# ctu-mrs/vofod

Measured on AMD Instinct MI355X. Metric: LiDAR frames/sec (131k-pt OS1-128) at 1/2/4/8 MI355X + HBM roofline %, higher is better.
Workload: dtype f32; 1 GPU; os1-128 128x1024 scans, 0.25 m voxels, batched process_scan (configs[1] scan shape in configs[3]'s batched form); points_per_frame=131072, map_voxels=19480981, map_warm_scans=96, gpu_max_hw_queues=4

## Files before the change

### vofod_amd/csrc/kernels_classify.h

```cpp
#pragma once
#include <hip/hip_runtime.h>

#include "common.h"

namespace vc
{
using namespace vk;

constexpr int EX_MAX_R = 32;
constexpr int EX_SIDE = 2 * EX_MAX_R + 1;
constexpr uint32_t EX_CELLS = EX_SIDE * EX_SIDE * EX_SIDE;
constexpr uint32_t EX_WORDS = (EX_CELLS + 31) / 32;
constexpr uint32_t EX_MAX_JOBS = 1024;

struct ExploreJob
{
  uint32_t frame;
  uint32_t n_members;
  uint32_t member_off;
  int32_t R;
  int32_t box_lo[3], box_hi[3];
  uint32_t result_slot;
};

struct ExploreResult
{
  uint32_t floating;
  uint32_t overflow;
  double conf_sum;
};

struct ExploreParams
{
  float thr_unknown, thr_ground, frontier_value;
  double ray_score;
  int32_t no_update;
  uint32_t stack_cap;
};

__device__ __forceinline__ void wave_sync()
{
  __builtin_amdgcn_fence(__ATOMIC_RELEASE, "workgroup");
  __builtin_amdgcn_wave_barrier();
  __builtin_amdgcn_fence(__ATOMIC_ACQUIRE, "workgroup");
}

__device__ __forceinline__ uint32_t pack_rel(int dx, int dy, int dz) { return static_cast<uint32_t>((dx + 128) | ((dy + 128) << 8) | ((dz + 128) << 16)); }

__device__ __forceinline__ void explore_frame(const ExploreParams& ep, const MapGeom& mg, const ExploreJob* __restrict__ jobs, const uint32_t jb, const uint32_t je, const int* __restrict__ members,
                                              float* __restrict__ map, unsigned long long* __restrict__ overlay_all, uint32_t* __restrict__ stack_all, uint32_t* __restrict__ explored_all,
                                              uint32_t* __restrict__ touched_all, uint32_t* __restrict__ ovl_list_all, uint32_t* __restrict__ ovl_count_all, ExploreResult* __restrict__ results,
                                              uint32_t* __restrict__ visited_all, const uint32_t slot, uint8_t* s_float, uint8_t* s_walk)
{
  const int lane = threadIdx.x & 63;
  if (jb == je)
    return;
  const uint64_t ovl_words = (mg.n + 63) >> 6;
  unsigned long long* overlay = overlay_all + static_cast<uint64_t>(slot) * ovl_words;
  uint32_t* stack = stack_all + static_cast<uint64_t>(slot) * ep.stack_cap;
  uint32_t* explored = explored_all + static_cast<uint64_t>(slot) * ep.stack_cap;
  uint32_t* ovl_list = ovl_list_all + static_cast<uint64_t>(slot) * ep.stack_cap;
  uint32_t* touched = touched_all + static_cast<uint64_t>(slot) * ep.stack_cap;
  uint32_t* visited = visited_all + static_cast<uint64_t>(slot) * EX_WORDS;

  auto map_read = [&](uint64_t li) -> float {
    const float mv = map[li];
    if (!ep.no_update)
      return mv;
    const unsigned long long ow = __hip_atomic_load(&overlay[li >> 6], __ATOMIC_RELAXED, __HIP_MEMORY_SCOPE_AGENT);
    return ((ow >> (li & 63)) & 1ull) ? ep.frontier_value : mv;
  };

  for (uint32_t j = jb; j < je; j++)
  {
    const ExploreJob job = jobs[j];
    bool floating = true;
    uint32_t overflow = 0;
    const float max_voxel_dist = static_cast<float>(job.R);
    uint32_t m = 0;
    while (m < job.n_members && floating)
    {
      {
        const uint32_t mm = m + lane;
        int kind = 0;
        if (mm < job.n_members)
        {
          const int sx_ = members[3 * (job.member_off + mm)], sy_ = members[3 * (job.member_off + mm) + 1], sz_ = members[3 * (job.member_off + mm) + 2];
          if (sx_ <= 0 || sy_ <= 0 || sz_ <= 0 || sx_ >= mg.sx - 1 || sy_ >= mg.sy - 1 || sz_ >= mg.sz - 1)
            kind = 1;
          else
          {
            const float sv = map_read((static_cast<uint64_t>(sz_) * mg.sy + sy_) * mg.sx + sx_);
            kind = sv > ep.thr_ground ? 1 : (sv > ep.thr_unknown ? 2 : 0);
          }
        }
        const unsigned long long need = __ballot(kind != 0);
        if (!need)
        {
          m += 64;
          continue;
        }
        const int first = __ffsll(static_cast<long long>(need)) - 1;
        m += first;
        if (__shfl(kind, first) == 1)
        {
          floating = false;
          break;
        }
      }
      const int ox = members[3 * (job.member_off + m)], oy = members[3 * (job.member_off + m) + 1], oz = members[3 * (job.member_off + m) + 2];
      if (job.R - 1 >= 1 && job.R - 1 <= 31)
      {
        const int len = job.R - 1;
        float wv[3];
        bool win[3];
        const uint64_t li0 = (static_cast<uint64_t>(oz) * mg.sy + oy) * mg.sx + ox;
#pragma unroll
        for (int u = 0; u < 3; u++)
        {
          const int e = lane + 64 * u, q = e >> 5, d = (e & 31) + 1;
          const int ax = ox + (q == 0 ? d : q == 3 ? -d : 0), ay = oy + (q == 1 ? d : q == 4 ? -d : 0), az = oz + (q == 2 ? d : q == 5 ? -d : 0);
          win[u] = d <= len && ax >= 0 && ax <= mg.sx - 1 && ay >= 0 && ay <= mg.sy - 1 && az >= 0 && az <= mg.sz - 1;
          wv[u] = map_read(win[u] ? (static_cast<uint64_t>(az) * mg.sy + ay) * mg.sx + ax : li0);
        }
#pragma unroll
        for (int u = 0; u < 3; u++)
          s_walk[lane + 64 * u] = !win[u] ? 0 : (wv[u] > ep.thr_ground ? 2 : (wv[u] > ep.thr_unknown ? 1 : 0));
        wave_sync();
        bool walk_ok = false;
        if (lane < 6)
        {
          walk_ok = true;
          for (int d = 1; d <= len; d++)
          {
            const uint8_t st = s_walk[(lane << 5) + d - 1];
            if (st == 2)
              break;
            if (st == 0)
            {
              walk_ok = false;
              break;
            }
          }
        }
        const bool any_walk = __ballot(walk_ok) != 0ull;
        wave_sync();
        if (any_walk)
        {
          floating = false;
          break;
        }
      }
      uint32_t n_stack = 1, n_expl = 0, n_touched = 1;
      if (lane == 0)
      {
        stack[0] = pack_rel(0, 0, 0);
        const uint32_t c = (EX_MAX_R * EX_SIDE + EX_MAX_R) * EX_SIDE + EX_MAX_R;
        atomicOr(&visited[c >> 5], 1u << (c & 31));
        touched[0] = c;
      }
      wave_sync();
      bool connected = false;
      while (n_stack > 0 && !connected)
      {
        const uint32_t take = min(n_stack, 64u);
        const uint32_t base = n_stack - take;
        n_stack = base;
        bool have = static_cast<uint32_t>(lane) < take;
        int dx = 0, dy = 0, dz = 0;
        float val = 0.0f;
        if (have)
        {
          const uint32_t e = stack[base + lane];
          dx = static_cast<int>(e & 255u) - 128;
          dy = static_cast<int>((e >> 8) & 255u) - 128;
          dz = static_cast<int>((e >> 16) & 255u) - 128;
          val = map_read((static_cast<uint64_t>(oz + dz) * mg.sy + (oy + dy)) * mg.sx + (ox + dx));
        }
        const bool ground = have && val > ep.thr_ground;
        const bool unknown = have && !ground && val > ep.thr_unknown;
        const int md = abs(dx) + abs(dy) + abs(dz);
        const bool rim = unknown && static_cast<float>(md) == max_voxel_dist - 1.0f;
        if (__ballot(ground || rim))
        {
          connected = true;
          break;
        }
        const unsigned long long um = __ballot(unknown);
        if (unknown)
        {
          const uint32_t pos = n_expl + __popcll(um & ((1ull << lane) - 1ull));
          if (pos < ep.stack_cap)
            explored[pos] = pack_rel(dx, dy, dz);
        }
        n_expl += __popcll(um);
        uint32_t mine[6];
        int n_mine = 0;
        if (unknown)
        {
          const int nb[6][3] = {{1, 0, 0}, {0, 1, 0}, {0, 0, 1}, {-1, 0, 0}, {0, -1, 0}, {0, 0, -1}};
          uint32_t oldw[6], bitq[6];
          bool okq[6];
#pragma unroll
          for (int q = 0; q < 6; q++)
          {
            const int tx = dx + nb[q][0], ty = dy + nb[q][1], tz = dz + nb[q][2];
            const int ax = ox + tx, ay = oy + ty, az = oz + tz;
            const int tmd = abs(tx) + abs(ty) + abs(tz);
            okq[q] = !(ax < 0 || ax > mg.sx - 1 || ay < 0 || ay > mg.sy - 1 || az < 0 || az > mg.sz - 1) && static_cast<float>(tmd) <= max_voxel_dist;
            const uint32_t c = okq[q] ? ((tz + EX_MAX_R) * EX_SIDE + (ty + EX_MAX_R)) * EX_SIDE + (tx + EX_MAX_R) : 0u;
            bitq[q] = 1u << (c & 31);
            oldw[q] = okq[q] ? atomicOr(&visited[c >> 5], bitq[q]) : 0xffffffffu;
          }
#pragma unroll
          for (int q = 0; q < 6; q++)
            if (okq[q] && !(oldw[q] & bitq[q]))
              mine[n_mine++] = pack_rel(dx + nb[q][0], dy + nb[q][1], dz + nb[q][2]);
        }
        uint32_t incl = static_cast<uint32_t>(n_mine);
#pragma unroll
        for (int s = 1; s < 64; s <<= 1)
        {
          const uint32_t t = __shfl_up(incl, s);
          if (lane >= s)
            incl += t;
        }
        const uint32_t total = __shfl(incl, 63);
        uint32_t at = n_stack + incl - n_mine;
        uint32_t tat = n_touched + incl - n_mine;
        for (int q = 0; q < n_mine; q++, at++, tat++)
        {
          if (at < ep.stack_cap)
            stack[at] = mine[q];
          else
            overflow = 1;
          if (tat < ep.stack_cap)
          {
            const int tx = static_cast<int>(mine[q] & 255u) - 128, ty = static_cast<int>((mine[q] >> 8) & 255u) - 128, tz = static_cast<int>((mine[q] >> 16) & 255u) - 128;
            touched[tat] = ((tz + EX_MAX_R) * EX_SIDE + (ty + EX_MAX_R)) * EX_SIDE + (tx + EX_MAX_R);
          }
        }
        n_stack = min(n_stack + total, ep.stack_cap);
        n_touched += total;
        wave_sync();
      }
      wave_sync();
      if (n_touched <= ep.stack_cap)
      {
        for (uint32_t e = lane; e < n_touched; e += 64)
          __hip_atomic_store(&visited[touched[e] >> 5], 0u, __ATOMIC_RELAXED, __HIP_MEMORY_SCOPE_AGENT);
      }
      else
        for (uint32_t w = lane; w < EX_WORDS; w += 64)
          __hip_atomic_store(&visited[w], 0u, __ATOMIC_RELAXED, __HIP_MEMORY_SCOPE_AGENT);
      __threadfence_block();
      wave_sync();
      if (connected)
      {
        floating = false;
        break;
      }
      for (uint32_t e = lane; e < min(n_expl, ep.stack_cap); e += 64)
      {
        const uint32_t pk = explored[e];
        const int dx = static_cast<int>(pk & 255u) - 128, dy = static_cast<int>((pk >> 8) & 255u) - 128, dz = static_cast<int>((pk >> 16) & 255u) - 128;
        const uint64_t li = (static_cast<uint64_t>(oz + dz) * mg.sy + (oy + dy)) * mg.sx + (ox + dx);
        if (ep.no_update)
        {
          const unsigned long long bit = 1ull << (li & 63);
          const unsigned long long old = atomicOr(&overlay[li >> 6], bit);
          if (!(old & bit))
          {
            const uint32_t pos = atomicAdd(&ovl_count_all[slot], 1u);
            if (pos < ep.stack_cap)
              ovl_list[pos] = static_cast<uint32_t>(li >> 6);
          }
        }
        else
          map[li] = ep.frontier_value;
      }
      __threadfence_block();
      wave_sync();
      m++;
    }
    if (lane == 0)
    {
      s_float[j - jb] = floating ? 1 : 0;
      results[job.result_slot].floating = floating ? 1u : 0u;
      results[job.result_slot].overflow = overflow;
      results[job.result_slot].conf_sum = 0.0;
    }
  }
  __threadfence_block();
  wave_sync();

  for (uint32_t j = jb; j < je; j++)
  {
    const ExploreJob job = jobs[j];
    if (!s_float[j - jb])
      continue;
    const int nx = job.box_hi[0] - job.box_lo[0] + 1, ny = job.box_hi[1] - job.box_lo[1] + 1, nz = job.box_hi[2] - job.box_lo[2] + 1;
    const uint32_t cells = static_cast<uint32_t>(nx) * ny * nz;
    double acc = 0.0;
    for (uint32_t c = lane; c < cells; c += 64)
    {
      const int x = job.box_lo[0] + static_cast<int>(c % nx), y = job.box_lo[1] + static_cast<int>((c / nx) % ny), z = job.box_lo[2] + static_cast<int>(c / (nx * ny));
      bool is_member = false;
      for (uint32_t m = 0; m < job.n_members; m++)
      {
        const int* o = &members[3 * (job.member_off + m)];
        is_member |= (o[0] == x && o[1] == y && o[2] == z);
      }
      const float v = is_member ? static_cast<float>(ep.ray_score) : map_read((static_cast<uint64_t>(z) * mg.sy + y) * mg.sx + x);
      acc += 1.0 - static_cast<double>(v) / ep.ray_score;
    }
#pragma unroll
    for (int s = 32; s > 0; s >>= 1)
      acc += __shfl_xor(acc, s);
    if (lane == 0)
      results[job.result_slot].conf_sum = acc;
  }
  if (ep.no_update)
  {
    wave_sync();
    const uint32_t n = __hip_atomic_load(&ovl_count_all[slot], __ATOMIC_RELAXED, __HIP_MEMORY_SCOPE_AGENT);
    if (n <= ep.stack_cap)
      for (uint32_t e = lane; e < n; e += 64)
        overlay[ovl_list[e]] = 0ull;
    else
      for (uint64_t w = lane; w < ovl_words; w += 64)
        overlay[w] = 0ull;
    wave_sync();
    if (lane == 0)
      ovl_count_all[slot] = 0;
  }
}

__global__ __attribute__((amdgpu_waves_per_eu(8, 8))) __launch_bounds__(64) void k_explore(const ExploreParams ep, const MapGeom mg, const ExploreJob* __restrict__ jobs, const uint32_t* __restrict__ job_begin, const uint32_t* __restrict__ job_end,
                                                const int* __restrict__ members, float* __restrict__ map, unsigned long long* __restrict__ overlay_all,
                                                uint32_t* __restrict__ stack_all, uint32_t* __restrict__ explored_all, uint32_t* __restrict__ touched_all,
                                                uint32_t* __restrict__ ovl_list_all, uint32_t* __restrict__ ovl_count_all, ExploreResult* __restrict__ results, uint32_t* __restrict__ visited_all)
{
  __shared__ uint8_t s_float[EX_MAX_JOBS];
  __shared__ uint8_t s_walk[6 * 32];
  const uint32_t slot = blockIdx.x;
  explore_frame(ep, mg, jobs, job_begin[slot], job_end[slot], members, map, overlay_all, stack_all, explored_all, touched_all, ovl_list_all, ovl_count_all, results, visited_all, slot, s_float, s_walk);
}

}
```

### vofod_amd/csrc/kernels_tail.h

```cpp
#pragma once
#include <hip/hip_runtime.h>

#include "host_tail.h"
#include "kernels_classify.h"
#include "kernels_voxelize.h"

namespace vtd
{

#ifndef TAIL_WPB_DEF
#define TAIL_WPB_DEF 8
#endif
constexpr int TAIL_WPB = TAIL_WPB_DEF;
#if TAIL_WPB_DEF >= 16
#define TAIL_OCC_ATTR
#else
#define TAIL_OCC_ATTR __attribute__((amdgpu_waves_per_eu(5, 5)))
#endif
using namespace vk;

constexpr int TAIL_STAGE = 512;
constexpr int TP_THREADS = 256;
constexpr int TP_MAXM = TAIL_MAXM;
constexpr int TP_MAXC = TAIL_MAXC;
constexpr int TP_MAXD = 16;

using vt::TailParams;

struct TailCluster
{
  uint32_t root, n_members;
  float obb_center[3];
  int32_t job;
};

struct DetRaw
{
  uint32_t root, n_points;
  float center[3];
  uint32_t pad;
  double conf_sum;
};

struct FrameDets
{
  uint32_t n;
  uint32_t fallback;
  int32_t status;
  uint32_t n_jobs;
  DetRaw d[TP_MAXD];
};

enum : uint32_t { TAIL_FB_MEMBERS = 1u, TAIL_FB_CLUSTERS = 2u, TAIL_FB_RADIUS = 4u, TAIL_FB_DETS = 8u, TAIL_FB_EXPLORE = 16u };

__device__ __forceinline__ uint32_t rank_in_wave(bool flag, int lane, uint32_t& count)
{
  const unsigned long long m = __ballot(flag);
  count = __popcll(m);
  return __popcll(m & ((1ull << lane) - 1ull));
}

__device__ __forceinline__ void put_header(FrameDets& out, FrameDets* hout, uint32_t f, uint32_t n, uint32_t fb, int32_t status, uint32_t n_jobs)
{
  out.n = n;
  out.fallback = fb;
  out.status = status;
  out.n_jobs = n_jobs;
  if (hout)
  {
    hout[f].n = n;
    hout[f].fallback = fb;
    hout[f].status = status;
    hout[f].n_jobs = n_jobs;
  }
}

__device__ __forceinline__ void write_records(const TailCluster& tc, const vc::ExploreResult* __restrict__ results, int lane, FrameDets& out, FrameDets* hout, uint32_t f, uint32_t& n, uint32_t& fb)
{
  bool det = false, bad = false;
  double conf = 0.0;
  if (tc.job >= 0)
  {
    const vc::ExploreResult r = results[tc.job];
    det = r.floating != 0u;
    bad = r.overflow != 0u;
    conf = r.conf_sum;
  }
  const uint32_t pos = rank_in_wave(det, lane, n);
  const unsigned long long bm = __ballot(bad);
  if (det && pos < TP_MAXD)
  {
    DetRaw d;
    d.root = tc.root;
    d.n_points = tc.n_members;
    for (int q = 0; q < 3; q++)
      d.center[q] = tc.obb_center[q];
    d.pad = 0;
    d.conf_sum = conf;
    out.d[pos] = d;
    if (hout)
      hout[f].d[pos] = d;
  }
  fb = (n > TP_MAXD ? TAIL_FB_DETS : 0u) | (bm ? TAIL_FB_EXPLORE : 0u);
}

template <class Get>
__device__ __forceinline__ bool gate_cluster(uint32_t f, uint32_t m_begin, uint32_t m_count, Get get, const float* tf, const MapGeom& mg, const TailParams& tp, int* __restrict__ members_out, TailCluster& tc,
                                             vc::ExploreJob& job, uint32_t& fallback)
{
  const int s3[3] = {mg.sx, mg.sy, mg.sz};
  const vt::Gates gt = vt::classify_gates(m_count, get, tf, tp, mg.off, mg.vs_inv, s3);
  for (int q = 0; q < 3; q++)
    tc.obb_center[q] = gt.obb_center[q];
  if (!gt.explore)
    return false;
  job.frame = f;
  job.n_members = m_count;
  job.member_off = f * TP_MAXM + m_begin;
  job.R = gt.R;
  if (job.R > vc::EX_MAX_R || job.R < 0)
    fallback |= TAIL_FB_RADIUS;
  for (int q = 0; q < 3; q++)
  {
    job.box_lo[q] = gt.box_lo[q];
    job.box_hi[q] = gt.box_hi[q];
  }
  for (uint32_t i = 0; i < m_count; i++)
  {
    float p[3];
    get(i, p);
    int* o = members_out + 3 * static_cast<size_t>(job.member_off + i);
    for (int q = 0; q < 3; q++)
      o[q] = vt::map_cell(p[q], mg.off[q], mg.vs_inv);
  }
  return true;
}

__global__ __launch_bounds__(TP_THREADS) void k_tail_prep(const GridParams g, const FrameHdr* __restrict__ hdrs, const FrameArgs* __restrict__ args, const ClusterRec* __restrict__ table_all,
                                                         const CandMember* __restrict__ cand_all, VoxelArrays va_all, const MapGeom mg, const TailParams tp, vc::ExploreJob* __restrict__ jobs,
                                                         uint32_t* __restrict__ job_begin, uint32_t* __restrict__ job_end, int* __restrict__ members_out, TailCluster* __restrict__ tailc,
                                                         FrameDets* __restrict__ dets)
{
  __shared__ unsigned long long s_key[TP_MAXM];
  __shared__ ClusterRec s_rec[TP_MAXC];
  __shared__ uint32_t s_ord[TP_MAXC];
  __shared__ uint32_t s_nc;
  const uint32_t f = blockIdx.x;
  const FrameHdr h = hdrs[f];
  const int tid = threadIdx.x;
  FrameDets& out = dets[f];
  uint32_t fallback = 0;
  if (tid == 0)
  {
    s_nc = 0;
    job_begin[f] = f * TP_MAXC;
    job_end[f] = f * TP_MAXC;
  }
  __syncthreads();
  const uint32_t n_cand = h.status == VOFOD_OK ? h.n_cand : 0u;
  const uint32_t C = h.status == VOFOD_OK ? h.C : 0u;
  if (n_cand > TP_MAXM)
    fallback |= TAIL_FB_MEMBERS;
  const ClusterRec* table = table_all + static_cast<size_t>(f) * g.vox_cap;
  for (uint32_t c = tid; c < C; c += TP_THREADS)
  {
    const ClusterRec r = table[c];
    if (r.cand && !r.close)
    {
      const uint32_t pos = atomicAdd(&s_nc, 1u);
      if (pos < TP_MAXC)
        s_rec[pos] = r;
    }
  }
  uint32_t np2 = 1;
  while (np2 < n_cand && np2 < TP_MAXM)
    np2 <<= 1;
  const CandMember* cands = cand_all + static_cast<size_t>(f) * g.vox_cap;
  if (!(fallback & TAIL_FB_MEMBERS))
    for (uint32_t i = tid; i < np2; i += TP_THREADS)
    {
      unsigned long long k = ~0ull;
      if (i < n_cand)
      {
        const CandMember cm = cands[i];
        k = (static_cast<unsigned long long>(cm.root) << 32) | cm.v;
      }
      s_key[i] = k;
    }
  __syncthreads();
  if (!(fallback & TAIL_FB_MEMBERS) && n_cand > 1)
    for (uint32_t k = 2; k <= np2; k <<= 1)
      for (uint32_t j = k >> 1; j > 0; j >>= 1)
      {
        for (uint32_t i = tid; i < np2; i += TP_THREADS)
        {
          const uint32_t l = i ^ j;
          if (l > i)
          {
            const unsigned long long a = s_key[i], b = s_key[l];
            const bool up = (i & k) == 0;
            if ((a > b) == up)
            {
              s_key[i] = b;
              s_key[l] = a;
            }
          }
        }
        __syncthreads();
      }
  const uint32_t nc_all = s_nc;
  if (nc_all > TP_MAXC)
    fallback |= TAIL_FB_CLUSTERS;
  const uint32_t nc = fallback ? 0u : nc_all;
  if (tid < static_cast<int>(nc))
  {
    const ClusterRec me = s_rec[tid];
    uint32_t rank = 0;
    for (uint32_t j = 0; j < nc; j++)
    {
      const ClusterRec o = s_rec[j];
      rank += (o.size > me.size || (o.size == me.size && o.root < me.root)) ? 1u : 0u;
    }
    s_ord[rank] = tid;
  }
  __syncthreads();
  if (tid >= 64)
    return;
  const int lane = tid;
  bool live = lane < static_cast<int>(nc);
  const VoxelArrays va = frame_voxels(va_all, f, g.vox_cap);
  const FrameArgs& a = args[f];
  bool wants_job = false;
  vc::ExploreJob job{};
  TailCluster tc{};
  tc.job = -1;
  uint32_t m_begin = 0, m_count = 0;
  if (live)
  {
    const ClusterRec rec = s_rec[s_ord[lane]];
    tc.root = rec.root;
    uint32_t lo = 0, hi = n_cand;
    const unsigned long long want = static_cast<unsigned long long>(rec.root) << 32;
    while (lo < hi)
    {
      const uint32_t mid = (lo + hi) >> 1;
      if (s_key[mid] < want)
        lo = mid + 1;
      else
        hi = mid;
    }
    m_begin = lo;
    while (m_begin + m_count < n_cand && static_cast<uint32_t>(s_key[m_begin + m_count] >> 32) == rec.root)
      m_count++;
    tc.n_members = m_count;
    auto get = [&](size_t i, float p[3]) {
      const float4 q = va.pts[static_cast<uint32_t>(s_key[m_begin + i])];
      p[0] = q.x;
      p[1] = q.y;
      p[2] = q.z;
    };
    wants_job = gate_cluster(f, m_begin, m_count, get, a.tf, mg, tp, members_out, tc, job, fallback);
  }
  uint32_t n_jobs;
  const uint32_t slot = f * TP_MAXC + rank_in_wave(wants_job, lane, n_jobs);
  if (wants_job)
  {
    job.result_slot = slot;
    jobs[slot] = job;
    tc.job = static_cast<int32_t>(slot);
  }
  uint32_t fb_all = fallback;
#pragma unroll
  for (int s = 32; s > 0; s >>= 1)
    fb_all |= __shfl_xor(fb_all, s);
  if (live)
    tailc[f * TP_MAXC + lane] = tc;
  if (lane == 0)
  {
    put_header(out, nullptr, f, 0u, fb_all, h.status, fb_all ? 0u : n_jobs);
    if (!fb_all)
      job_end[f] = f * TP_MAXC + n_jobs;
  }
  if (!live && lane < TP_MAXC)
  {
    TailCluster e{};
    e.job = -1;
    tailc[f * TP_MAXC + lane] = e;
  }
}

__global__ TAIL_OCC_ATTR __launch_bounds__(64 * TAIL_WPB) void k_tail_far(const GridParams g, const FrameHdr* __restrict__ hdrs, const FrameArgs* __restrict__ args, const ClusterRec* __restrict__ table_all,
                                                const CandMember* __restrict__ cand_all, VoxelArrays va_all, const MapGeom mg, const TailParams tp, const vc::ExploreParams ep, vc::ExploreJob* __restrict__ jobs,
                                                int* __restrict__ members_out, float* __restrict__ map, unsigned long long* __restrict__ overlay_all, uint32_t* __restrict__ stack_all,
                                                uint32_t* __restrict__ explored_all, uint32_t* __restrict__ touched_all, uint32_t* __restrict__ ovl_list_all, uint32_t* __restrict__ ovl_count_all,
                                                vc::ExploreResult* __restrict__ results, uint32_t* __restrict__ visited_all, FrameDets* __restrict__ dets, FrameDets* __restrict__ hout,
                                                TailCluster* __restrict__ tailc, unsigned long long* __restrict__ prof)
{
  __shared__ uint8_t s_float_all[TAIL_WPB][TP_MAXC];
  __shared__ uint8_t s_walk_all[TAIL_WPB][6 * 32];
  __shared__ float s_pts_all[TAIL_WPB][TAIL_STAGE][3];
  const uint32_t f = blockIdx.x * TAIL_WPB + (threadIdx.x >> 6);
  if (f >= g.n_frames)
    return;
  uint8_t* s_float = s_float_all[threadIdx.x >> 6];
  uint8_t* s_walk = s_walk_all[threadIdx.x >> 6];
  const FrameHdr h = hdrs[f];
  const int lane = threadIdx.x & 63;
  const unsigned long long tp0 = prof ? wall_clock64() : 0ull;
  unsigned long long tp1 = 0ull, tp2 = 0ull;
  FrameDets& out = dets[f];
  uint32_t fallback = 0;
  const bool ok = h.status == VOFOD_OK;
  const uint32_t n_cand = ok ? h.n_cand : 0u;
  const uint32_t nc_all = ok ? h.n_cand_clusters : 0u;
  if (n_cand > static_cast<uint32_t>(TP_MAXM))
    fallback |= TAIL_FB_MEMBERS;
  if (nc_all > static_cast<uint32_t>(TP_MAXC))
    fallback |= TAIL_FB_CLUSTERS;
  const uint32_t nc = fallback ? 0u : nc_all;
  const bool live = lane < static_cast<int>(nc);
  const ClusterRec* table = table_all + static_cast<size_t>(f) * g.vox_cap;
  const CandMember* cands = cand_all + static_cast<size_t>(f) * g.vox_cap;
  const VoxelArrays va = frame_voxels(va_all, f, g.vox_cap);
  const FrameArgs& a = args[f];
  ClusterRec rec{};
  if (live)
    rec = table[lane];
  uint32_t m_count = live ? rec.size : 0u, m_begin = 0;
  {
    uint32_t incl = m_count;
#pragma unroll
    for (int s = 1; s < 64; s <<= 1)
    {
      const uint32_t t = __shfl_up(incl, s);
      if (lane >= s)
        incl += t;
    }
    m_begin = incl - m_count;
  }
  float (*s_pts)[3] = s_pts_all[threadIdx.x >> 6];
  {
    const uint32_t total = min(static_cast<uint32_t>(__shfl(m_begin + m_count, 63)), static_cast<uint32_t>(TAIL_STAGE));
    for (uint32_t i = lane; i < total; i += 64)
    {
      const float4 q = va.pts[cands[i].v];
      s_pts[i][0] = q.x;
      s_pts[i][1] = q.y;
      s_pts[i][2] = q.z;
    }
    vc::wave_sync();
  }
  bool wants_job = false;
  vc::ExploreJob job{};
  TailCluster tc{};
  tc.job = -1;
  if (live)
  {
    tc.root = rec.root;
    tc.n_members = m_count;
    auto get = [&](size_t i, float p[3]) {
      const uint32_t k = m_begin + static_cast<uint32_t>(i);
      if (k < static_cast<uint32_t>(TAIL_STAGE))
      {
        p[0] = s_pts[k][0];
        p[1] = s_pts[k][1];
        p[2] = s_pts[k][2];
        return;
      }
      const float4 q = va.pts[cands[k].v];
      p[0] = q.x;
      p[1] = q.y;
      p[2] = q.z;
    };
    wants_job = gate_cluster(f, m_begin, m_count, get, a.tf, mg, tp, members_out, tc, job, fallback);
  }
  uint32_t n_jobs;
  const uint32_t jb = f * TP_MAXC;
  const uint32_t slot = jb + rank_in_wave(wants_job, lane, n_jobs);
  if (wants_job)
  {
    job.result_slot = slot;
    jobs[slot] = job;
    tc.job = static_cast<int32_t>(slot);
  }
  if (tailc)
  {
    if (!live)
    {
      tc = TailCluster{};
      tc.job = -1;
    }
    tailc[f * TP_MAXC + lane] = tc;
  }
  uint32_t fb_all = fallback;
#pragma unroll
  for (int s = 32; s > 0; s >>= 1)
    fb_all |= __shfl_xor(fb_all, s);
  if (fb_all)
  {
    if (lane == 0)
      put_header(out, hout, f, 0u, fb_all, h.status, 0u);
    return;
  }
  __threadfence_block();
  vc::wave_sync();
  if (prof)
    tp1 = wall_clock64();
  vc::explore_frame(ep, mg, jobs, jb, jb + n_jobs, members_out, map, overlay_all, stack_all, explored_all, touched_all, ovl_list_all, ovl_count_all, results, visited_all, f, s_float, s_walk);
  __threadfence_block();
  vc::wave_sync();
  if (prof)
    tp2 = wall_clock64();
  uint32_t n, fb;
  write_records(tc, results, lane, out, hout, f, n, fb);
  if (lane == 0)
  {
    put_header(out, hout, f, n, fb, h.status, n_jobs);
    if (prof)
    {
      const unsigned long long te = wall_clock64();
      auto d20 = [&](unsigned long long t) { return (t - tp0) > 0xfffffull ? 0xfffffull : (t - tp0); };
      prof[static_cast<size_t>(f) * 32 + 22] = tp0;
      prof[static_cast<size_t>(f) * 32 + 23] = d20(tp1) | (d20(tp2) << 20) | (d20(te) << 40) | (static_cast<unsigned long long>(n_jobs > 15u ? 15u : n_jobs) << 60);
    }
  }
}

__global__ __launch_bounds__(64) void k_tail_finish(const TailCluster* __restrict__ tailc, const vc::ExploreResult* __restrict__ results, FrameDets* __restrict__ dets, FrameDets* __restrict__ hout)
{
  const uint32_t f = blockIdx.x;
  const int lane = threadIdx.x;
  FrameDets& out = dets[f];
  const uint32_t fb_in = out.fallback;
  if (fb_in)
  {
    if (lane == 0)
      put_header(out, hout, f, 0u, fb_in, out.status, out.n_jobs);
    return;
  }
  const TailCluster tc = tailc[f * TP_MAXC + lane];
  uint32_t n, fb;
  write_records(tc, results, lane, out, hout, f, n, fb);
  if (lane == 0)
    put_header(out, hout, f, n, fb, out.status, out.n_jobs);
}

}
```

Measured before the change: 1.327 million frames/s.

## Cache flood-fill stack window in LDS and classify neighbors at push time

```diff
diff --git a/vofod_amd/csrc/kernels_classify.h b/vofod_amd/csrc/kernels_classify.h
--- a/vofod_amd/csrc/kernels_classify.h
+++ b/vofod_amd/csrc/kernels_classify.h
@@ -12,6 +12,9 @@
 constexpr uint32_t EX_CELLS = EX_SIDE * EX_SIDE * EX_SIDE;
 constexpr uint32_t EX_WORDS = (EX_CELLS + 31) / 32;
 constexpr uint32_t EX_MAX_JOBS = 1024;
+constexpr uint32_t EX_WIN = 512;
+constexpr uint32_t EX_KIND_NEITHER = 0, EX_KIND_UNKNOWN = 1, EX_KIND_GROUND = 2;
+static_assert((EX_WIN & (EX_WIN - 1)) == 0 && EX_WIN >= 6 * 64, "a round pushes up to 6 * 64 entries: none of them may land on another of the same round");
 
 struct ExploreJob
 {
@@ -45,12 +48,25 @@
   __builtin_amdgcn_fence(__ATOMIC_ACQUIRE, "workgroup");
 }
 
+__device__ __forceinline__ void wave_sync_lds()
+{
+  __builtin_amdgcn_fence(__ATOMIC_RELEASE, "wavefront");
+  __builtin_amdgcn_wave_barrier();
+  __builtin_amdgcn_fence(__ATOMIC_ACQUIRE, "wavefront");
+}
+
+__device__ __forceinline__ void wave_sync_stores()
+{
+  __builtin_amdgcn_s_waitcnt(0x0f70);
+  wave_sync();
+}
+
 __device__ __forceinline__ uint32_t pack_rel(int dx, int dy, int dz) { return static_cast<uint32_t>((dx + 128) | ((dy + 128) << 8) | ((dz + 128) << 16)); }
 
 __device__ __forceinline__ void explore_frame(const ExploreParams& ep, const MapGeom& mg, const ExploreJob* __restrict__ jobs, const uint32_t jb, const uint32_t je, const int* __restrict__ members,
                                               float* __restrict__ map, unsigned long long* __restrict__ overlay_all, uint32_t* __restrict__ stack_all, uint32_t* __restrict__ explored_all,
                                               uint32_t* __restrict__ touched_all, uint32_t* __restrict__ ovl_list_all, uint32_t* __restrict__ ovl_count_all, ExploreResult* __restrict__ results,
-                                              uint32_t* __restrict__ visited_all, const uint32_t slot, uint8_t* s_float, uint8_t* s_walk)
+                                              uint32_t* __restrict__ visited_all, const uint32_t slot, uint8_t* s_float, uint8_t* s_walk, uint32_t* s_stack)
 {
   const int lane = threadIdx.x & 63;
   if (jb == je)
@@ -152,33 +168,40 @@
         }
       }
       uint32_t n_stack = 1, n_expl = 0, n_touched = 1;
+      uint32_t wm = 0;
       if (lane == 0)
       {
-        stack[0] = pack_rel(0, 0, 0);
+        const uint32_t e0 = pack_rel(0, 0, 0) | (EX_KIND_UNKNOWN << 24);
+        stack[0] = e0;
+        s_stack[0] = e0;
         const uint32_t c = (EX_MAX_R * EX_SIDE + EX_MAX_R) * EX_SIDE + EX_MAX_R;
         atomicOr(&visited[c >> 5], 1u << (c & 31));
         touched[0] = c;
       }
-      wave_sync();
+      wave_sync_stores();
       bool connected = false;
       while (n_stack > 0 && !connected)
       {
         const uint32_t take = min(n_stack, 64u);
         const uint32_t base = n_stack - take;
         n_stack = base;
-        bool have = static_cast<uint32_t>(lane) < take;
-        int dx = 0, dy = 0, dz = 0;
-        float val = 0.0f;
-        if (have)
-        {
-          const uint32_t e = stack[base + lane];
-          dx = static_cast<int>(e & 255u) - 128;
-          dy = static_cast<int>((e >> 8) & 255u) - 128;
-          dz = static_cast<int>((e >> 16) & 255u) - 128;
-          val = map_read((static_cast<uint64_t>(oz + dz) * mg.sy + (oy + dy)) * mg.sx + (ox + dx));
-        }
-        const bool ground = have && val > ep.thr_ground;
-        const bool unknown = have && !ground && val > ep.thr_unknown;
+        const bool have = static_cast<uint32_t>(lane) < take;
+        uint32_t e = 0;
+        if (have && base + lane >= wm)
+          e = s_stack[(base + lane) & (EX_WIN - 1)];
+        if (base < wm)
+        {
+          wave_sync_stores();
+          uint32_t eg = 0;
+          if (have && base + lane < wm)
+            eg = stack[base + lane];
+          e |= eg;
+          wm = base;
+        }
+        const int dx = static_cast<int>(e & 255u) - 128, dy = static_cast<int>((e >> 8) & 255u) - 128, dz = static_cast<int>((e >> 16) & 255u) - 128;
+        const uint32_t kd = (e >> 24) & 3u;
+        const bool ground = have && kd == EX_KIND_GROUND;
+        const bool unknown = have && kd == EX_KIND_UNKNOWN;
         const int md = abs(dx) + abs(dy) + abs(dz);
         const bool rim = unknown && static_cast<float>(md) == max_voxel_dist - 1.0f;
         if (__ballot(ground || rim))
@@ -187,37 +210,51 @@
           break;
         }
         const unsigned long long um = __ballot(unknown);
-        if (unknown)
-        {
-          const uint32_t pos = n_expl + __popcll(um & ((1ull << lane) - 1ull));
-          if (pos < ep.stack_cap)
-            explored[pos] = pack_rel(dx, dy, dz);
-        }
+        const uint32_t epos = n_expl + __popcll(um & ((1ull << lane) - 1ull));
         n_expl += __popcll(um);
         uint32_t mine[6];
-        int n_mine = 0;
+        uint32_t newm = 0;
         if (unknown)
         {
           const int nb[6][3] = {{1, 0, 0}, {0, 1, 0}, {0, 0, 1}, {-1, 0, 0}, {0, -1, 0}, {0, 0, -1}};
           uint32_t oldw[6], bitq[6];
-          bool okq[6];
+          float mv[6];
+          unsigned long long ow[6];
+          uint32_t osh[6];
+          uint32_t okm = 0;
 #pragma unroll
           for (int q = 0; q < 6; q++)
           {
             const int tx = dx + nb[q][0], ty = dy + nb[q][1], tz = dz + nb[q][2];
             const int ax = ox + tx, ay = oy + ty, az = oz + tz;
             const int tmd = abs(tx) + abs(ty) + abs(tz);
-            okq[q] = !(ax < 0 || ax > mg.sx - 1 || ay < 0 || ay > mg.sy - 1 || az < 0 || az > mg.sz - 1) && static_cast<float>(tmd) <= max_voxel_dist;
-            const uint32_t c = okq[q] ? ((tz + EX_MAX_R) * EX_SIDE + (ty + EX_MAX_R)) * EX_SIDE + (tx + EX_MAX_R) : 0u;
-            bitq[q] = 1u << (c & 31);
-            oldw[q] = okq[q] ? atomicOr(&visited[c >> 5], bitq[q]) : 0xffffffffu;
-          }
+            const bool okq = !(ax < 0 || ax > mg.sx - 1 || ay < 0 || ay > mg.sy - 1 || az < 0 || az > mg.sz - 1) && static_cast<float>(tmd) <= max_voxel_dist;
+            if (okq)
+            {
+              okm |= 1u << q;
+              const uint32_t c = ((tz + EX_MAX_R) * EX_SIDE + (ty + EX_MAX_R)) * EX_SIDE + (tx + EX_MAX_R);
+              const uint64_t li = (static_cast<uint64_t>(az) * mg.sy + ay) * mg.sx + ax;
+              bitq[q] = 1u << (c & 31);
+              oldw[q] = atomicOr(&visited[c >> 5], bitq[q]);
+              mv[q] = map[li];
+              osh[q] = static_cast<uint32_t>(li) & 63u;
+              if (ep.no_update)
+                ow[q] = __hip_atomic_load(&overlay[li >> 6], __ATOMIC_RELAXED, __HIP_MEMORY_SCOPE_AGENT);
+            }
+          }
+          __builtin_amdgcn_s_waitcnt(0x0f70);
 #pragma unroll
           for (int q = 0; q < 6; q++)
-            if (okq[q] && !(oldw[q] & bitq[q]))
-              mine[n_mine++] = pack_rel(dx + nb[q][0], dy + nb[q][1], dz + nb[q][2]);
-        }
-        uint32_t incl = static_cast<uint32_t>(n_mine);
+            if ((okm & (1u << q)) && !(oldw[q] & bitq[q]))
+            {
+              const float v = ep.no_update && ((ow[q] >> osh[q]) & 1ull) ? ep.frontier_value : mv[q];
+              const uint32_t k = v > ep.thr_ground ? EX_KIND_GROUND : (v > ep.thr_unknown ? EX_KIND_UNKNOWN : EX_KIND_NEITHER);
+              mine[q] = pack_rel(dx + nb[q][0], dy + nb[q][1], dz + nb[q][2]) | (k << 24);
+              newm |= 1u << q;
+            }
+        }
+        const uint32_t n_mine = __popc(newm);
+        uint32_t incl = n_mine;
 #pragma unroll
         for (int s = 1; s < 64; s <<= 1)
         {
@@ -225,26 +262,37 @@
           if (lane >= s)
             incl += t;
         }
-        const uint32_t total = __shfl(incl, 63);
+        const uint32_t total = __builtin_amdgcn_readlane(incl, 63);
+        if (unknown && epos < ep.stack_cap)
+          explored[epos] = pack_rel(dx, dy, dz);
         uint32_t at = n_stack + incl - n_mine;
         uint32_t tat = n_touched + incl - n_mine;
-        for (int q = 0; q < n_mine; q++, at++, tat++)
-        {
-          if (at < ep.stack_cap)
-            stack[at] = mine[q];
-          else
-            overflow = 1;
-          if (tat < ep.stack_cap)
-          {
-            const int tx = static_cast<int>(mine[q] & 255u) - 128, ty = static_cast<int>((mine[q] >> 8) & 255u) - 128, tz = static_cast<int>((mine[q] >> 16) & 255u) - 128;
-            touched[tat] = ((tz + EX_MAX_R) * EX_SIDE + (ty + EX_MAX_R)) * EX_SIDE + (tx + EX_MAX_R);
-          }
-        }
+#pragma unroll
+        for (int q = 0; q < 6; q++)
+          if (newm & (1u << q))
+          {
+            if (at < ep.stack_cap)
+            {
+              s_stack[at & (EX_WIN - 1)] = mine[q];
+              stack[at] = mine[q];
+            }
+            else
+              overflow = 1;
+            if (tat < ep.stack_cap)
+            {
+              const int tx = static_cast<int>(mine[q] & 255u) - 128, ty = static_cast<int>((mine[q] >> 8) & 255u) - 128, tz = static_cast<int>((mine[q] >> 16) & 255u) - 128;
+              touched[tat] = ((tz + EX_MAX_R) * EX_SIDE + (ty + EX_MAX_R)) * EX_SIDE + (tx + EX_MAX_R);
+            }
+            at++;
+            tat++;
+          }
         n_stack = min(n_stack + total, ep.stack_cap);
         n_touched += total;
-        wave_sync();
-      }
-      wave_sync();
+        if (n_stack > wm + EX_WIN)
+          wm = n_stack - EX_WIN;
+        wave_sync_lds();
+      }
+      wave_sync_stores();
       if (n_touched <= ep.stack_cap)
       {
         for (uint32_t e = lane; e < n_touched; e += 64)
@@ -336,15 +384,16 @@
   }
 }
 
-__global__ __attribute__((amdgpu_waves_per_eu(8, 8))) __launch_bounds__(64) void k_explore(const ExploreParams ep, const MapGeom mg, const ExploreJob* __restrict__ jobs, const uint32_t* __restrict__ job_begin, const uint32_t* __restrict__ job_end,
+__global__ __attribute__((amdgpu_waves_per_eu(4, 8))) __launch_bounds__(64) void k_explore(const ExploreParams ep, const MapGeom mg, const ExploreJob* __restrict__ jobs, const uint32_t* __restrict__ job_begin, const uint32_t* __restrict__ job_end,
                                                 const int* __restrict__ members, float* __restrict__ map, unsigned long long* __restrict__ overlay_all,
                                                 uint32_t* __restrict__ stack_all, uint32_t* __restrict__ explored_all, uint32_t* __restrict__ touched_all,
                                                 uint32_t* __restrict__ ovl_list_all, uint32_t* __restrict__ ovl_count_all, ExploreResult* __restrict__ results, uint32_t* __restrict__ visited_all)
 {
   __shared__ uint8_t s_float[EX_MAX_JOBS];
   __shared__ uint8_t s_walk[6 * 32];
+  __shared__ uint32_t s_stack[EX_WIN];
   const uint32_t slot = blockIdx.x;
-  explore_frame(ep, mg, jobs, job_begin[slot], job_end[slot], members, map, overlay_all, stack_all, explored_all, touched_all, ovl_list_all, ovl_count_all, results, visited_all, slot, s_float, s_walk);
-}
-
-}
+  explore_frame(ep, mg, jobs, job_begin[slot], job_end[slot], members, map, overlay_all, stack_all, explored_all, touched_all, ovl_list_all, ovl_count_all, results, visited_all, slot, s_float, s_walk, s_stack);
+}
+
+}
diff --git a/vofod_amd/csrc/kernels_tail.h b/vofod_amd/csrc/kernels_tail.h
--- a/vofod_amd/csrc/kernels_tail.h
+++ b/vofod_amd/csrc/kernels_tail.h
@@ -12,11 +12,6 @@
 #define TAIL_WPB_DEF 8
 #endif
 constexpr int TAIL_WPB = TAIL_WPB_DEF;
-#if TAIL_WPB_DEF >= 16
-#define TAIL_OCC_ATTR
-#else
-#define TAIL_OCC_ATTR __attribute__((amdgpu_waves_per_eu(5, 5)))
-#endif
 using namespace vk;
 
 constexpr int TAIL_STAGE = 512;
@@ -289,7 +284,7 @@
   }
 }
 
-__global__ TAIL_OCC_ATTR __launch_bounds__(64 * TAIL_WPB) void k_tail_far(const GridParams g, const FrameHdr* __restrict__ hdrs, const FrameArgs* __restrict__ args, const ClusterRec* __restrict__ table_all,
+__global__ __launch_bounds__(64 * TAIL_WPB) void k_tail_far(const GridParams g, const FrameHdr* __restrict__ hdrs, const FrameArgs* __restrict__ args, const ClusterRec* __restrict__ table_all,
                                                 const CandMember* __restrict__ cand_all, VoxelArrays va_all, const MapGeom mg, const TailParams tp, const vc::ExploreParams ep, vc::ExploreJob* __restrict__ jobs,
                                                 int* __restrict__ members_out, float* __restrict__ map, unsigned long long* __restrict__ overlay_all, uint32_t* __restrict__ stack_all,
                                                 uint32_t* __restrict__ explored_all, uint32_t* __restrict__ touched_all, uint32_t* __restrict__ ovl_list_all, uint32_t* __restrict__ ovl_count_all,
@@ -299,6 +294,7 @@
   __shared__ uint8_t s_float_all[TAIL_WPB][TP_MAXC];
   __shared__ uint8_t s_walk_all[TAIL_WPB][6 * 32];
   __shared__ float s_pts_all[TAIL_WPB][TAIL_STAGE][3];
+  __shared__ uint32_t s_stack_all[TAIL_WPB][vc::EX_WIN];
   const uint32_t f = blockIdx.x * TAIL_WPB + (threadIdx.x >> 6);
   if (f >= g.n_frames)
     return;
@@ -406,7 +402,7 @@
   vc::wave_sync();
   if (prof)
     tp1 = wall_clock64();
-  vc::explore_frame(ep, mg, jobs, jb, jb + n_jobs, members_out, map, overlay_all, stack_all, explored_all, touched_all, ovl_list_all, ovl_count_all, results, visited_all, f, s_float, s_walk);
+  vc::explore_frame(ep, mg, jobs, jb, jb + n_jobs, members_out, map, overlay_all, stack_all, explored_all, touched_all, ovl_list_all, ovl_count_all, results, visited_all, f, s_float, s_walk, s_stack_all[threadIdx.x >> 6]);
   __threadfence_block();
   vc::wave_sync();
   if (prof)
```

Result: slower. 1.314 million frames/s (-1.0%).
